# SKIRT/SKIRT9

Hardware: AMD Instinct MI355X
Metric: photon packets/s (whole node), 10^6-cell octree (higher is better)
Workload: dtype f64

## Files before the change

### include/pmc_tuning.h

```cpp
#ifndef PMC_TUNING_H
#define PMC_TUNING_H

#include "pmc.h"

#ifdef __cplusplus
extern "C" {
#endif

int pmc_tuning_set(const char* name, const char* value);
void pmc_tuning_clear(void);

int pmc_set_launch(pmc_ctx* ctx, int32_t block, int32_t grid);

typedef struct pmc_walk_work_values
{
    uint64_t peel_wave_steps, peel_lane_steps, peel_rounds;
    uint64_t prop_wave_steps, prop_lane_steps, prop_rounds;
} pmc_walk_work_values;
int pmc_walk_work(pmc_ctx* ctx, pmc_walk_work_values* out);
typedef struct pmc_debug_table_values
{
    const void* cell_table;
    int64_t cell_slots;
    int64_t loose_base;
    const int32_t* task_cell;
    int64_t num_slots;
} pmc_debug_table_values;
int pmc_debug_tables(pmc_ctx* ctx, pmc_debug_table_values* out);

int pmc_launch_flavour(pmc_ctx* ctx, int32_t* flavour);

int pmc_tune_dipole_cosines(pmc_ctx* ctx, const double* u, int64_t n, double* cos_out);

int pmc_tune_source_velocities(pmc_ctx* ctx, int32_t source, const double* r, int64_t n, double* v_out);


typedef struct pmc_log_geometry_values
{
    int64_t cell_slots, rf_num_lambda, rf_keys, rf_parts, rf_logged;
    int64_t stat_records, stat_parts, stat_logged;
    int64_t chunk, rf_bucket_bits, stat_bucket_bits, scan_threads, sort_block, max_parts, reduce_span, rf_short_run, stat_short_run, max_entries;
} pmc_log_geometry_values;
int pmc_tune_log_geometry(pmc_ctx* ctx, pmc_log_geometry_values* out);

int pmc_tune_log_partition(pmc_ctx* ctx, int32_t stat, int32_t num_parts, const uint32_t* keys, const double* vals, const uint32_t* fills, int64_t n,
                           uint32_t* sorted_keys, double* sorted_vals, uint64_t* start);

int pmc_tune_rf_log_flush(pmc_ctx* ctx, const uint32_t* keys, const double* vals, int64_t n);

int pmc_tune_stat_log_flush(pmc_ctx* ctx, const uint32_t* keys, const double* vals, const uint32_t* fills, int64_t n, double* acc_out);

int pmc_tune_cell_numbering(pmc_ctx* ctx, int32_t* ext_out);


enum
{
    PMC_FN_HG_VALUE = 0,
    PMC_FN_HG_CONE_MEAN = 1,
    PMC_FN_PHASE_VALUE = 2,
    PMC_FN_HG_COSINE = 3,
    PMC_FN_DIPOLE_VALUE = 4,
    PMC_FN_RANDOM_DIRECTION = 5,
    PMC_FN_DIRECTION_ABOUT = 6,
// ... 57 lines not shown
```

### skirt9_amd/csrc/pmc_api.hip

```cpp
#include "pmc_context.h"
#include "pmc_scene_build.h"
#include <memory>

namespace
{
    thread_local std::string t_error;
    constexpr int MAX_DEVICES = 64;
    bool g_slotUsed[MAX_DEVICES][PMC_MAX_CONTEXTS] = {{false}};
    std::mutex g_slotMutex;
}

void pmcSetError(const std::string& message)
{
    t_error = message;
}


extern "C" {

int pmc_abi_version(void)
{
    return PMC_ABI_VERSION;
}

// ... 1 lines not shown
#define PMC_STRINGIFY(x) PMC_STRINGIFY2(x)
#ifndef PMC_BUILD_FLAGS
#define PMC_BUILD_FLAGS "unknown (not built by the Makefile)"
#endif
const char* pmc_build_info(void)
{
    return "libpmc ABI " PMC_STRINGIFY(PMC_ABI_VERSION) ", gfx950, " __VERSION__ ", flags: " PMC_BUILD_FLAGS
#if defined(__FP_FAST_FMA) || defined(__FAST_MATH__)
           " [fast-math macros defined]"
#endif
        ;
}

namespace
{
    __global__ void contractionProbeKernel(double a, double b, double c, double* out) { out[0] = a * b + c; }

    int checkContraction(int device)
    {
        static std::mutex m;
        static bool checked[64] = {false};
        std::lock_guard<std::mutex> lock(m);
        if (device >= 0 && device < 64 && checked[device]) return PMC_OK;
        double* d = nullptr;
        double h = 1.;
        if (hipMalloc(&d, sizeof(double)) != hipSuccess) return fail(PMC_ERR_DEVICE, "hipMalloc failed");
        hipLaunchKernelGGL(contractionProbeKernel, dim3(1), dim3(1), 0, 0, 1. + 0x1p-30, 1. - 0x1p-30, -1., d);
        const hipError_t e = hipMemcpy(&h, d, sizeof(double), hipMemcpyDeviceToHost);
        hipFree(d);
        if (e != hipSuccess) return hipFail(e, "contraction self-test");
        if (h != 0.)
            return fail(PMC_ERR_DEVICE, std::string("this libpmc.so was compiled with floating-point contraction (a * b + c fused): its results would differ from "
                                                    "the reference's in the last bits everywhere; rebuild with -ffp-contract=off.  ") + pmc_build_info());
        if (device >= 0 && device < 64) checked[device] = true;
        return PMC_OK;
    }
}

const char* pmc_last_error(void)
{
    return t_error.c_str();
}

int64_t pmc_frame_layout_of(const pmc_scene* scene, int32_t instrument, pmc_frame_layout* out)
{
    if (!scene) return fail(PMC_ERR_INVALID, "null scene");
    return pmc_layout_compute(scene, instrument, out);
}

void pmc_destroy(pmc_ctx* ctx)
{
    if (!ctx) return;
    hipSetDevice(ctx->device);
    for (int g = 0; g < PMC_MAX_GROUPS; ++g)
    {
        if (ctx->groupStream[g]) hipStreamSynchronize(ctx->groupStream[g]);
        if (ctx->peelStream[g]) hipStreamSynchronize(ctx->peelStream[g]);
    }
    for (void* p : ctx->allocations) hipFree(p);
    for (void* p : ctx->slotAllocations) hipFree(p);
    for (void* p : ctx->segmentAllocations) hipFree(p);
    if (ctx->readback) hipHostFree(ctx->readback);
    for (hipEvent_t e : {ctx->evStart, ctx->evStop})
        if (e) hipEventDestroy(e);
    for (int g = 0; g < PMC_MAX_GROUPS; ++g)
    {
        for (hipEvent_t e : {ctx->evA[g], ctx->evB[g], ctx->evC[g], ctx->evJoin[g], ctx->evProp[g]})
            if (e) hipEventDestroy(e);
        if (g > 0 && ctx->groupStream[g]) hipStreamDestroy(ctx->groupStream[g]);
        if (ctx->peelStream[g]) hipStreamDestroy(ctx->peelStream[g]);
    }
    if (ctx->stream) hipStreamDestroy(ctx->stream);
    if (ctx->slot >= 0)
    {
        std::lock_guard<std::mutex> lock(g_slotMutex);
        g_slotUsed[ctx->device][ctx->slot] = false;
    }
    delete ctx;
}

}

namespace
{
    SceneSwitches readSceneSwitches()
    {
        SceneSwitches sw;
        sw.treeAsBinTree = pmcTune("PMC_TREE_AS_BINTREE") != nullptr;
        sw.noMono = pmcTune("PMC_NO_MONO") != nullptr;
        sw.propNoCheckpoints = pmcTune("PMC_PROP_NO_CHECKPOINTS") != nullptr;
        sw.voroNoPeelKernel = pmcTune("PMC_VORO_NO_PEEL_KERNEL") != nullptr;
        sw.voroNoDeferredScan = pmcTune("PMC_VORO_NO_DEFERRED_SCAN") != nullptr;
        sw.voroNoCull = pmcTune("PMC_VORO_NO_CULL") != nullptr;
        sw.voroNoPropKernel = pmcTune("PMC_VORO_NO_PROP_KERNEL") != nullptr;
        sw.voroNoConeTables = pmcTune("PMC_VORO_NO_CONE_TABLES") != nullptr;
        sw.voroNoObserverLists = pmcTune("PMC_VORO_NO_OBSERVER_LISTS") != nullptr;
        sw.voroConeCullOnly = pmcTune("PMC_VORO_CONE_CULL_ONLY") != nullptr;
        if (const char* v = pmcTune("PMC_VORO_LINK_COUNT_MAX")) sw.voroLinkCountMax = std::min<uint32_t>(sw.voroLinkCountMax, (uint32_t)std::max(0, atoi(v)));
        if (const char* v = pmcTune("PMC_CELL_ORDER")) sw.cellOrderRef = !strcmp(v, "ref");
        if (const char* v = pmcTune("PMC_CELL_SHUFFLE")) sw.cellShuffle = atoi(v);
        if (const char* v = pmcTune("PMC_WALK_BLOCKS_PER_CU")) sw.walkBlocksPerCU = std::max(1, atoi(v));
        if (const char* v = pmcTune("PMC_PEEL_BLOCKS_PER_CU")) sw.peelBlocksPerCU = std::max(1, atoi(v));
        return sw;
    }

    struct DestroyContext
    {
        void operator()(pmc_ctx* ctx) const { pmc_destroy(ctx); }
    };
    using ContextPtr = std::unique_ptr<pmc_ctx, DestroyContext>;

    int makeContext(int device, ContextPtr& made)
    {
        if (device >= MAX_DEVICES) return fail(PMC_ERR_UNSUPPORTED, "device index beyond the context table");
        ContextPtr ctx(new pmc_ctx());
        ctx->device = device;
        {
            std::lock_guard<std::mutex> lock(g_slotMutex);
            for (int sl = 0; sl < PMC_MAX_CONTEXTS && ctx->slot < 0; ++sl)
                if (!g_slotUsed[device][sl])
                {
                    g_slotUsed[device][sl] = true;
                    ctx->slot = sl;
                }
        }
        if (ctx->slot < 0) return fail(PMC_ERR_NOMEM, "too many live pmc contexts (at most " + std::to_string(PMC_MAX_CONTEXTS) + ")");
        auto makeStream = [](hipStream_t* out) { return hipStreamCreateWithPriority(out, hipStreamDefault, 0); };
        if (makeStream(&ctx->stream) != hipSuccess) return fail(PMC_ERR_DEVICE, "hipStreamCreate failed");
        ctx->groupStream[0] = ctx->stream;
        for (int g = 1; g < PMC_MAX_GROUPS; ++g)
            if (makeStream(&ctx->groupStream[g]) != hipSuccess) return fail(PMC_ERR_DEVICE, "hipStreamCreate failed");
        for (int g = 0; g < PMC_MAX_GROUPS; ++g)
            if (makeStream(&ctx->peelStream[g]) != hipSuccess) return fail(PMC_ERR_DEVICE, "hipStreamCreate failed");
        for (hipEvent_t* ev : {&ctx->evStart, &ctx->evStop})
            if (hipEventCreate(ev) != hipSuccess) return fail(PMC_ERR_DEVICE, "hipEventCreate failed");
        for (int g = 0; g < PMC_MAX_GROUPS; ++g)
            for (hipEvent_t* ev : {&ctx->evA[g], &ctx->evB[g], &ctx->evC[g], &ctx->evJoin[g], &ctx->evProp[g]})
                if (hipEventCreate(ev) != hipSuccess) return fail(PMC_ERR_DEVICE, "hipEventCreate failed");
        if (const char* env = getenv("PMC_NUM_GROUPS"))
        {
            ctx->numGroups = std::min(PMC_MAX_GROUPS, std::max(1, atoi(env)));
            ctx->groupsConfigured = true;
        }
        if (hipHostMalloc(reinterpret_cast<void**>(&ctx->readback), PMC_MAX_GROUPS * sizeof(GroupReadback)) != hipSuccess)
            return fail(PMC_ERR_DEVICE, "hipHostMalloc failed");
        made = std::move(ctx);
        return PMC_OK;
    }

    int configureDevice(pmc_ctx* ctx, const SceneSwitches& sw)
    {
        const DevScene& D = ctx->dev;
        if (pmcConfigureKernels(ctx->walkLds, ctx->launchLds) != hipSuccess) return fail(PMC_ERR_DEVICE, "hipFuncSetAttribute failed");
        hipDeviceProp_t prop;
        if (hipGetDeviceProperties(&prop, ctx->device) != hipSuccess) return fail(PMC_ERR_DEVICE, "hipGetDeviceProperties failed");
        ctx->numCU = prop.multiProcessorCount;
        ctx->block = 256;
        ctx->wide = D.grid_kind == PMC_GRID_OCTREE && D.lmax > 10;
        int perCU = pmcWalkBlocksPerCU(D.grid_kind, D.grid_kind == PMC_GRID_OCTREE ? 2 : 0, ctx->wide,
                                       D.grid_kind == PMC_GRID_OCTREE ? pmcPropBlock() : ctx->block, ctx->walkLds);
        if (perCU < 1) perCU = 1;
        if (sw.walkBlocksPerCU) perCU = std::min(perCU, sw.walkBlocksPerCU);
        else perCU = std::min(perCU, D.grid_kind == PMC_GRID_OCTREE ? 1 : 3);
        ctx->grid = ctx->numCU * perCU;
        if (D.grid_kind == PMC_GRID_OCTREE)
        {
            int peelPerCU = pmcWalkBlocksPerCU(D.grid_kind, 1, ctx->wide, pmcPeelBlock(), ctx->walkLds);
            peelPerCU = std::min(std::max(peelPerCU, 1), 1);
            if (sw.peelBlocksPerCU) peelPerCU = sw.peelBlocksPerCU;
            ctx->peelGrid = ctx->numCU * peelPerCU;
        }
        ctx->numSlots = 24 * 1024 * 1024;
        if (const char* env = getenv("PMC_NUM_SLOTS"))
        {
            ctx->numSlots = std::max<int64_t>(1024, atoll(env));
            ctx->slotsConfigured = true;
        }
        return PMC_OK;
    }
}

extern "C" {

int pmc_create(const pmc_scene* scene, int32_t device, pmc_ctx** out)
{
    return pmc_create_ext(scene, nullptr, device, out);
}

int pmc_create_ext(const pmc_scene* scene, const pmc_scene_ext* ext, int32_t device, pmc_ctx** out)
{
    if (!scene || !out) return fail(PMC_ERR_INVALID, "null argument");
    *out = nullptr;
    int rc = PMC_OK;
    SceneExtension extension;
    if ((rc = checkScene(*scene, ext, extension))) return rc;
    if (pmcExperimentBuild())
    {
        static std::atomic<bool> said{false};
        if (!said.exchange(true)) fprintf(stderr, "libpmc: this library was built with an ablation / perturbation macro (a tuning experiment): its results are NOT those of the engine\n");
    }
    int count = 0;
    if (hipGetDeviceCount(&count) != hipSuccess || count < 1)
        return fail(PMC_ERR_DEVICE, "no HIP device available: the MI355X engine cannot run (there is no CPU fallback)");
    if (device < 0 || device >= count) return fail(PMC_ERR_INVALID, "invalid device index");
    HIP_TRY(hipSetDevice(device));
    if ((rc = checkContraction(device))) return rc;

    ContextPtr ctx;
    if ((rc = makeContext(device, ctx))) return rc;
    const SceneSwitches switches = readSceneSwitches();
    SceneTables tables;
    if ((rc = buildSceneTables(*scene, extension, switches, *ctx, ctx->dev, tables))) return rc;
    ctx->frameSize = tables.frameSize;
    ctx->rfSize = tables.rfSize;
    ctx->frames = ctx->dev.frames;
    ctx->walkLds = tables.lds.walkBytes, ctx->transitionLds = tables.lds.transitionBytes, ctx->launchLds = tables.lds.launchBytes;
    if ((rc = configureDevice(ctx.get(), switches))) return rc;
    *out = ctx.release();
    return PMC_OK;
}

int pmc_set_launch(pmc_ctx* ctx, int32_t block, int32_t grid)
{
    if (!ctx) return fail(PMC_ERR_INVALID, "null context");
    if (block > 0)
    {
        if (block % 64 || block > 256) return fail(PMC_ERR_INVALID, "block must be a multiple of 64 and at most 256");
        ctx->block = block;
    }
    if (grid > 0) ctx->grid = grid;
    return PMC_OK;
}

int pmc_set_num_slots(pmc_ctx* ctx, int64_t num_slots)
{
    if (!ctx) return fail(PMC_ERR_INVALID, "null context");
    if (num_slots < 1 || num_slots > (int64_t(1) << 30)) return fail(PMC_ERR_INVALID, "num_slots out of range");
    ctx->numSlots = num_slots;
    ctx->slotsConfigured = true;
    return PMC_OK;
}

int pmc_bind_frames(pmc_ctx* ctx, double* device_ptr, int64_t num_doubles)
{
    if (!ctx || !device_ptr) return fail(PMC_ERR_INVALID, "null argument");
    if (num_doubles != ctx->frameSize) return fail(PMC_ERR_INVALID, "frame buffer size mismatch");
    ctx->frames = device_ptr;
    ctx->dev.frames = device_ptr;
    ctx->sceneDirty = true;
    return PMC_OK;
}

int pmc_clear_frames(pmc_ctx* ctx)
{
    if (!ctx) return fail(PMC_ERR_INVALID, "null context");
    HIP_TRY(hipSetDevice(ctx->device));
    HIP_TRY(hipMemsetAsync(ctx->frames, 0, size_t(ctx->frameSize) * sizeof(double), ctx->stream));
    return PMC_OK;
}

int pmc_set_progress(pmc_ctx* ctx, pmc_progress_fn report, void* user, double interval_seconds)
{
    if (!ctx) return fail(PMC_ERR_INVALID, "null context");
    ctx->progress = report;
    ctx->progressUser = user;
    ctx->progressInterval = interval_seconds > 0. ? interval_seconds : 0.;
    return PMC_OK;
}

int pmc_sync(pmc_ctx* ctx)
{
    if (!ctx) return fail(PMC_ERR_INVALID, "null context");
    HIP_TRY(hipSetDevice(ctx->device));
    HIP_TRY(hipStreamSynchronize(ctx->stream));
    return PMC_OK;
}

int pmc_last_kernel_ms(pmc_ctx* ctx, float* ms)
{
    if (!ctx || !ms) return fail(PMC_ERR_INVALID, "null argument");
    if (!ctx->timed) return fail(PMC_ERR_INVALID, "no segment has been run yet");
    *ms = ctx->walkMs;
    return PMC_OK;
// ... 165 lines not shown
```

### skirt9_amd/csrc/pmc_context.h

```cpp
#ifndef PMC_CONTEXT_H
#define PMC_CONTEXT_H

#include "pmc_tables.h"
#include "../../include/pmc_layout.h"
#include "../../include/pmc_tuning.h"
#include <hip/hip_runtime.h>
#include <algorithm>
#include <chrono>
#include <cmath>
#include <cstdio>
#include <rccl/rccl.h>
#include <cstdlib>
#include <cstring>
#include <deque>
#include <atomic>
#include <mutex>
#include <string>
#include <thread>
#include <map>
#include <vector>

extern "C" const char* pmcTune(const char* name);
extern "C" hipError_t pmcUploadScene(int slot, const DevScene* scene, hipStream_t stream);
extern "C" hipError_t pmcConfigureKernels(size_t walkLds, size_t transitionLds);
// ... 28 lines not shown
extern "C" hipError_t pmcLaunchSourceVelocities(int slot, int source, const double* r, int64_t n, double* out, hipStream_t stream);
extern "C" hipError_t pmcLaunchDeviceFunction(int slot, int function, const double* args, int widthIn, int64_t n, double* out, int widthOut, hipStream_t stream);
extern "C" hipError_t pmcLaunchLocate(int kind, const double* nodes, int numNodes, const double* x, int64_t n, int32_t* out, hipStream_t stream);
extern "C" hipError_t pmcLaunchDetector(int slot, int instrument, const double* r, int64_t n, int32_t* pixel, int32_t* inside, hipStream_t stream);
extern "C" hipError_t pmcLaunchWavelengthBins(int slot, int instrument, const double* lambda, int64_t n, int32_t* ell, hipStream_t stream);
extern "C" hipError_t pmcLaunchAngularProbabilities(int slot, int source, const double* k, int64_t n, double* out, hipStream_t stream);
extern "C" hipError_t pmcLaunchTransition(int slot, int flavour, int slotBase, int numSlots, int group, uint64_t seed, const int* list, int listLen, int maxBlocks,
                                          size_t ldsBytes, const StatLogArgs* statLog, uint64_t count, hipStream_t stream);
extern "C" hipError_t pmcLaunchLaunch(int slot, int flavour, int slotBase, int numSlots, int group, uint64_t first, uint64_t count, uint64_t seed, int initial,
                                      int maxBlocks, size_t ldsBytes, const StatLogArgs* statLog, hipStream_t stream);
extern "C" hipError_t pmcLaunchStatFlush(int slot, const uint32_t* keys, const double* vals, uint32_t* sortedKeys, double* sortedVals, unsigned long long n,
                                         int numParts, void* temp, int numCU, const uint32_t* chunkFill, hipStream_t stream);
extern "C" int pmcStatBucketBits();
extern "C" void pmcLogConstants(pmc_log_geometry_values* out);
extern "C" hipError_t pmcLaunchLogPartition(int stat, const uint32_t* keys, const double* vals, uint32_t* sortedKeys, double* sortedVals, unsigned long long n,
                                            int numParts, void* temp, int numCU, const uint32_t* fills, hipStream_t stream);
extern "C" hipError_t pmcLaunchCycleStart(int slot, int gridKind, int kin, int slotBase, int numSlots, int listCounter, int* listOut, const int* listIn,
                                          int listLen, int maxBlocks, size_t ldsBytes, const PeelSortArgs* sort, hipStream_t stream);
extern "C" hipError_t pmcLaunchTrace(int slot, int gridKind, int wide, int uniform, const double r[3], const double k[3],
                                     const double* kdev, int32_t* m, double* ds, int32_t cap, int32_t* n, size_t ldsBytes,
                                     hipStream_t stream);
extern "C" int pmcProbeWorkWords(void);
extern "C" hipError_t pmcLaunchIntegrate(int slot, int gridKind, int wide, int averaged, const double* origins, const double* directions, const double* q,
                                         double* sums, unsigned long long numRays, unsigned long long* work, int grid, size_t ldsBytes, hipStream_t stream);
extern "C" hipError_t pmcLaunchLocateCells(int slot, int gridKind, int wide, const double* positions, int32_t* walkCells, int32_t* cells,
                                           unsigned long long numPoints, int grid, size_t ldsBytes, hipStream_t stream);
extern "C" hipError_t pmcLaunchGatherCells(const int32_t* walkCells, const double* q, double* values, unsigned long long numPoints, int numValues, int grid,
                                           hipStream_t stream);

namespace
{
    inline int hipFail(hipError_t e, const char* what)
    {
        return fail(PMC_ERR_DEVICE, std::string(what) + ": " + hipGetErrorString(e));
    }
}

#define HIP_TRY(call)                                           \
    do                                                          \
    {                                                           \
        hipError_t e_ = (call);                                 \
        if (e_ != hipSuccess) return hipFail(e_, #call);        \
    } while (0)

struct GroupReadback
{
    unsigned long long live;
    unsigned long long rfLogFill;
    unsigned long long statLogFill;
    unsigned long long historyCursor;
    unsigned long long statFreeBlocks;
};

struct pmc_ctx final : TableSink
{
    int device{0};
    int slot{-1};
    bool sceneDirty{true};
    hipStream_t stream{nullptr};
    int numGroups{3};
    hipStream_t groupStream[PMC_MAX_GROUPS]{};
    hipStream_t peelStream[PMC_MAX_GROUPS]{};
    hipEvent_t evA[PMC_MAX_GROUPS]{}, evB[PMC_MAX_GROUPS]{}, evC[PMC_MAX_GROUPS]{}, evJoin[PMC_MAX_GROUPS]{}, evProp[PMC_MAX_GROUPS]{};
    hipEvent_t evStart{nullptr}, evStop{nullptr};
    bool timed{false};
    float totalMs{0}, walkMs{0}, transitionMs{0};
    float peelMs{0}, propMs{0};
    int generations{0};
    float integrateMs{0};
    unsigned long long integrateLaneSteps{0}, integrateWaveSteps{0};
    float temperatureMs{0};
    float sampleMs{0};
    DevScene dev{};
    std::vector<void*> allocations;
    std::vector<void*> slotAllocations;
    double* frames{nullptr};
    int64_t frameSize{0};
    int64_t rfSize{0};
    size_t walkLds{0}, transitionLds{0}, launchLds{0};
    int block{256};
    int grid{0};
    int peelGrid{0};
    int wide{0};
    int numCU{256};
    int64_t numSlots{0};
    int64_t allocatedSlots{0};
    GroupReadback* readback{nullptr};
    unsigned long long internalErrorsSeen{0};
    pmc_progress_fn progress{nullptr};
    void* progressUser{nullptr};
    double progressInterval{3.};
    size_t steppedDownFree{0};
    bool slotsConfigured{false};
    bool groupsConfigured{false};
    unsigned long long overflowsSeen{0};
    int32_t* statPoolIota{nullptr};
    int64_t statPoolBlocks{0};
    int statPoolGrowths{0};
    std::vector<void*> segmentAllocations;
    uint32_t* rfKeys[PMC_MAX_GROUPS][2]{};
    double* rfVals[PMC_MAX_GROUPS][2]{};
    unsigned long long rfCap[PMC_MAX_GROUPS]{};
    void* rfTemp[PMC_MAX_GROUPS]{};
    PeelRec* peelRec[PMC_MAX_GROUPS][PMC_SORT_OBS]{};
    int32_t* peelList[PMC_MAX_GROUPS][PMC_SORT_OBS]{};
    void* peelTemp[PMC_MAX_GROUPS][PMC_SORT_OBS]{};
    unsigned long long* xcdCursors{nullptr};
    int peelCap[PMC_MAX_GROUPS]{};
    size_t rfTempBytes{0};
    uint32_t* statKeys[PMC_MAX_GROUPS][2]{};
    double* statVals[PMC_MAX_GROUPS][2]{};
    unsigned long long statCap[PMC_MAX_GROUPS]{};
    void* statTemp[PMC_MAX_GROUPS]{};
// ... 170 lines not shown
```

### skirt9_amd/csrc/pmc_run.hip

```cpp
#include "pmc_context.h"

namespace
{
    int allocateSlotArrays(pmc_ctx* ctx, int64_t n);
    void releaseSlots(pmc_ctx* ctx)
    {
        for (void* p : ctx->slotAllocations) hipFree(p);
        ctx->slotAllocations.clear();
        ctx->allocatedSlots = 0;
    }

    int allocateSlots(pmc_ctx* ctx, int64_t n)
    {
        hipSetDevice(ctx->device);
        releaseSlots(ctx);
        ctx->planning = true;
        ctx->plannedBytes = 0;
        int rc = allocateSlotArrays(ctx, n);
        ctx->planning = false;
        if (rc) return rc;
        size_t freeBytes = 0, totalBytes = 0;
        if (!ctx->slotsConfigured && n > (int64_t(1) << 20) && hipMemGetInfo(&freeBytes, &totalBytes) == hipSuccess && ctx->plannedBytes > freeBytes / 2)
        {
            const int64_t less = std::max<int64_t>(int64_t(1) << 20, n / 2);
// ... 154 lines not shown
        bool poolGrows;
        int statInstruments;
        int launchFlavour;
        int launchBlocks, cycleBlocks, transitionBlocks;
        int voroPropGrid, voroPeelGrid, voroPropSegments;
        bool serialWalks, genDump, xcdAffinity, voroPeelKernels, voroPropKernel, voroWalksInSeries;
    };
    struct SegmentRun
    {
        bool active[PMC_MAX_GROUPS], haveWalk[PMC_MAX_GROUPS];
        bool listBuilt[PMC_MAX_GROUPS];
        int listHalf[PMC_MAX_GROUPS];
        bool peelSorted[PMC_MAX_GROUPS];
        bool poolCannotGrow;
        float walkMs, transMs, peelMs, propMs;
        int generations;
    };

    int provisionSlots(pmc_ctx* ctx, uint64_t count, int* numSlots)
    {
        const int64_t want = std::min<int64_t>(ctx->numSlots, (int64_t)std::min<uint64_t>(count, uint64_t(1) << 30));
        bool grow = want > ctx->allocatedSlots;
        if (grow && ctx->allocatedSlots > 0 && ctx->steppedDownFree)
        {
            size_t freeBytes = 0, totalBytes = 0;
            grow = hipMemGetInfo(&freeBytes, &totalBytes) == hipSuccess && freeBytes > ctx->steppedDownFree + ctx->steppedDownFree / 4;
        }
        if (grow)
        {
            HIP_TRY(hipStreamSynchronize(ctx->stream));
            ctx->steppedDownFree = 0;
            int rc = allocateSlots(ctx, want);
            if (rc) return rc;
        }
        *numSlots = (int)std::min<int64_t>(want, ctx->allocatedSlots);
        HIP_TRY(sceneUpToDate(ctx));
        return PMC_OK;
    }

    int launchFlavour(const pmc_ctx* ctx)
    {
        const DevScene& D = ctx->dev;
        if (pmcTune("PMC_LAUNCH_GENERIC") != nullptr) return D.kin ? PMC_LAUNCH_KIN : 0;
        return pmcLaunchFlavourOf(D.src, D.num_sources, D.kin);
    }

    SegmentPlan planSegment(const pmc_ctx* ctx, int numSlots, uint64_t first, uint64_t count, uint64_t seed)
    {
        const DevScene& D = ctx->dev;
        SegmentPlan P;
        std::memset(&P, 0, sizeof(P));
        P.first = first, P.count = count, P.seed = seed;
        P.octree = D.grid_kind == PMC_GRID_OCTREE;
        P.serialWalks = pmcTune("PMC_SERIAL_WALKS") != nullptr;
        P.genDump = pmcTune("PMC_GEN_DUMP") != nullptr;
        const bool peelSort = pmcTune("PMC_NO_PEEL_SORT") == nullptr;
        int G = ctx->numGroups;
        if (numSlots < G * 65536) G = 1;
        {
            int observers = 0;
            for (int i = 0; i < D.num_instruments; ++i) observers += D.inst[i].same_observer ? 0 : 1;
            if (D.grid_kind == PMC_GRID_VORONOI && observers <= PMC_SORT_OBS && !ctx->groupsConfigured && peelSort) G = 1;
        }
        P.G = G;
        const int per = ((numSlots + G - 1) / G + PMC_TRANSITION_ALIGN - 1) / PMC_TRANSITION_ALIGN * PMC_TRANSITION_ALIGN;
        for (int g = 0; g < G; ++g)
        {
            P.base[g] = std::min(numSlots, g * per);
            P.size[g] = std::min(per, numSlots - P.base[g]);
        }
        P.walkFlavour = (D.rf_store ? 1 : 0) | (D.explicit_absorption ? 2 : 0) | (D.num_media > 1 ? 4 : 0);
        P.peelForm = (ctx->wide ? 1 : 0) | (D.num_media > 1 ? 2 : 0);
        if (pmcPeelHasQueues(P.peelForm, ctx->walkLds)) P.peelForm |= 4;
        P.propCheckpoints = pmcPropHasCheckpoints(P.walkFlavour, ctx->walkLds);
        P.propSortIndex = -1;
        if (peelSort && (!P.octree || (P.peelForm & 4)))
        {
            int observers = 0;
            for (int i = 0; i < D.num_instruments; ++i)
                if (!D.inst[i].same_observer)
                {
                    if (observers < PMC_SORT_OBS) P.sortObs[observers] = i;
                    ++observers;
                }
            if (observers <= PMC_SORT_OBS) P.numSortObs = observers;
        }
        if (!P.octree && P.numSortObs > 0 && P.numSortObs < PMC_SORT_OBS && pmcTune("PMC_NO_PROP_SORT") == nullptr) P.propSortIndex = P.numSortObs;
        P.numSortLists = P.numSortObs + (P.propSortIndex >= 0 ? 1 : 0);
        PeelSortArgs& sa = P.sortArgs;
        sa.numObs = P.numSortObs;
        sa.propIndex = P.propSortIndex;
        for (int i = 0; i < 16; ++i) sa.sortIndex[i] = -1;
        for (int k = 0; k < P.numSortObs; ++k) sa.obs[k] = P.sortObs[k], sa.sortIndex[P.sortObs[k]] = (int8_t)k;
        const double gdx = D.gx1 - D.gx0, gdy = D.gy1 - D.gy0, gdz = D.gz1 - D.gz0;
        sa.centre[0] = 0.5 * (D.gx0 + D.gx1), sa.centre[1] = 0.5 * (D.gy0 + D.gy1), sa.centre[2] = 0.5 * (D.gz0 + D.gz1);
        sa.scale = PMC_PEEL_TILES / std::sqrt(gdx * gdx + gdy * gdy + gdz * gdz);
        P.xcdAffinity = pmcTune("PMC_NO_XCD_AFFINITY") == nullptr;
        P.sparseLists = P.octree && pmcTune("PMC_NO_LIVE_LISTS") == nullptr;
        P.listTasksPerLane = 1;
        if (const char* env = pmcTune("PMC_LIST_TASKS_PER_LANE")) P.listTasksPerLane = std::max(1, atoi(env));
        P.voroPeelKernels = D.grid_kind == PMC_GRID_VORONOI && pmcTune("PMC_VORO_NO_PEEL_KERNEL") == nullptr;
        P.voroPropKernel = D.grid_kind == PMC_GRID_VORONOI && D.vgen_run && pmcTune("PMC_VORO_NO_PROP_KERNEL") == nullptr
                           && !(pmcTune("PMC_VORO_PLAIN_PROP_ONLY") && (D.num_media > 1 || D.rf_store || D.explicit_absorption));
        P.voroWalksInSeries = pmcTune("PMC_VORO_WALKS_IN_SERIES") != nullptr;
        P.voroPropSegments = (P.xcdAffinity && pmcTune("PMC_VPROP_XCD_SEGMENTS")) ? 8 : 1;
        int propBlocks = pmcVoroPropWavesPerSimd(), peelBlocks = pmcVoroPeelWavesPerSimd();
        if (const char* v = pmcTune("PMC_VPROP_BLOCKS_PER_CU")) propBlocks = std::max(1, atoi(v));
        if (const char* v = pmcTune("PMC_VPEEL_BLOCKS_PER_CU")) peelBlocks = std::max(1, atoi(v));
        P.voroPropGrid = ctx->numCU * propBlocks, P.voroPeelGrid = ctx->numCU * peelBlocks;
        const LogPlan logs = pmcLogPlan(ctx);
        P.rfLogged = logs.rfLogged;
        if (D.rf_store && P.octree && logs.rfParts > pmcRfMaxParts())
        {
            static std::atomic<bool> said{false};
            if (!said.exchange(true))
                fprintf(stderr, "libpmc: the radiation field table has %lld entries, more than the log's counting sort partitions (%d x %d): contributions are added atomically\n",
// ... 799 lines not shown
```

### skirt9_amd/engine.py

```python
import ctypes as C
import os

import numpy as np

from .host import AdaptiveMesh, CounterValues, DustHeating, FrameLayout, SceneExt, SceneHead, heating_struct, mesh_struct

_LIBDIR = os.path.join(os.path.dirname(os.path.abspath(__file__)), "lib")

SYMBOLS = ["pmc_abi_version", "pmc_build_info", "pmc_last_error", "pmc_frame_layout_of", "pmc_create", "pmc_create_ext", "pmc_destroy", "pmc_bind_frames",
           "pmc_clear_frames", "pmc_run_primary", "pmc_set_progress", "pmc_sync", "pmc_download", "pmc_frames_device", "pmc_frames_size",
           "pmc_last_kernel_ms", "pmc_counters", "pmc_reset_counters", "pmc_trace_ray", "pmc_integrate_rays",
           "pmc_last_integrate_work", "pmc_integrate_weighted_rays", "pmc_sample_cells", "pmc_last_sample_ms", "pmc_dust_temperatures",
           "pmc_last_temperature_ms", "pmc_set_launch",
           "pmc_set_num_slots", "pmc_last_timing", "pmc_last_walk_timing", "pmc_walk_work", "pmc_radiation_field_size", "pmc_radiation_field_device",
           "pmc_download_radiation_field", "pmc_clear_radiation_field", "pmc_bind_radiation_field", "pmc_sampler_create",
           "pmc_sampler_density", "pmc_sampler_destroy", "pmc_sampler_create_mesh", "pmc_history_range", "pmc_comm_init_all", "pmc_comm_unique_id",
           "pmc_comm_init_rank", "pmc_comm_size", "pmc_comm_destroy", "pmc_reduce_frames", "pmc_allreduce_radiation_field",
           "pmc_debug_tables", "pmc_tuning_set", "pmc_tuning_clear", "pmc_tune_dipole_cosines", "pmc_tune_source_velocities",
           "pmc_launch_flavour", "pmc_tune_log_geometry", "pmc_tune_log_partition", "pmc_tune_rf_log_flush", "pmc_tune_stat_log_flush",
           "pmc_tune_cell_numbering", "pmc_tune_device_function", "pmc_tune_device_function_widths", "pmc_tune_locate", "pmc_tune_instrument",
           "pmc_tune_detector", "pmc_tune_wavelength_bins", "pmc_tune_angular_probabilities", "pmc_tune_walk_cycle", "pmc_tune_walk_cycle_limits"]

DEVICE_FUNCTIONS = {"hg_value": 0, "hg_cone_mean": 1, "phase_value": 2, "hg_cosine": 3, "dipole_value": 4, "random_direction": 5, "direction_about": 6,
                    "lambert_lower_branch": 7, "generalized_exp": 8, "interpolate_loglog": 9, "lnmean": 10, "peel_taumax": 11, "shifted_wavelength": 12}
LOCATE_KINDS = {"locate": 0, "locate_clip": 1, "locate_basic": 2}

_lib = None


class DebugTables(C.Structure):
    _fields_ = [("cell_table", C.c_void_p), ("cell_slots", C.c_int64), ("loose_base", C.c_int64), ("task_cell", C.c_void_p), ("num_slots", C.c_int64)]


class WalkWork(C.Structure):
    _fields_ = [(n, C.c_uint64) for n in ("peel_wave_steps", "peel_lane_steps", "peel_rounds", "prop_wave_steps",
                                          "prop_lane_steps", "prop_rounds")]


class InstrumentValues(C.Structure):
    _fields_ = ([(n, C.c_double) for n in ("costheta", "sintheta", "cosphi", "sinphi", "cosomega", "sinomega", "xpmin", "xpsiz", "ypmin", "ypsiz",
                                           "aperture_r2", "zp1")]
                + [(n, C.c_int64) for n in ("nxp", "nyp", "num_border", "num_lambda", "include_sed", "include_ifu")])


class LogGeometry(C.Structure):
    _fields_ = [(n, C.c_int64) for n in ("cell_slots", "rf_num_lambda", "rf_keys", "rf_parts", "rf_logged", "stat_records", "stat_parts", "stat_logged",
                                         "chunk", "rf_bucket_bits", "stat_bucket_bits", "scan_threads", "sort_block", "max_parts", "reduce_span",
                                         "rf_short_run", "stat_short_run", "max_entries")]


class WalkCycleIn(C.Structure):
    _fields_ = ([("n", C.c_int64), ("live_list", C.c_int32)]
                + [(n, C.c_void_p) for n in ("list", "r", "k", "mask", "ppW", "u1", "u2", "depth", "hint", "nscatt", "wavelength", "dust_ext", "dust_sca",
                                             "dust_abs", "dust_idx", "W", "rfell")])


class WalkCycleOut(C.Structure):
    _fields_ = ([(n, C.c_void_p) for n in ("ptau", "sint", "nint", "mint", "taupath", "tausample")]
                + [(n, C.c_uint64) for n in ("visits", "rewalks", "paths", "internal_errors")])


def lib():
    global _lib
    if _lib is None:
        path = os.environ.get("PMC_LIBRARY") or os.path.join(_LIBDIR, "libpmc.so")
        if not os.path.exists(path):
            raise RuntimeError(f"{path} is missing: the HIP engine has not been built (run `make` or "
                               "__graft_entry__.build()); there is no CPU fallback")
        L = C.CDLL(path)
        L.pmc_abi_version.restype = C.c_int
        L.pmc_last_error.restype = C.c_char_p
        L.pmc_build_info.restype = C.c_char_p
        L.pmc_frame_layout_of.restype = C.c_int64
        L.pmc_frame_layout_of.argtypes = [C.c_void_p, C.c_int32, C.POINTER(FrameLayout)]
        L.pmc_create.argtypes = [C.c_void_p, C.c_int32, C.POINTER(C.c_void_p)]
        if hasattr(L, "pmc_create_ext"):
            L.pmc_create_ext.argtypes = [C.c_void_p, C.c_void_p, C.c_int32, C.POINTER(C.c_void_p)]
            L.pmc_tune_dipole_cosines.argtypes = [C.c_void_p, C.c_void_p, C.c_int64, C.c_void_p]
        if hasattr(L, "pmc_tune_source_velocities"):
            L.pmc_tune_source_velocities.argtypes = [C.c_void_p, C.c_int32, C.c_void_p, C.c_int64, C.c_void_p]
        L.pmc_destroy.argtypes = [C.c_void_p]
        L.pmc_bind_frames.argtypes = [C.c_void_p, C.c_void_p, C.c_int64]
        L.pmc_clear_frames.argtypes = [C.c_void_p]
        L.pmc_run_primary.argtypes = [C.c_void_p, C.c_uint64, C.c_uint64, C.c_uint64]
        L.pmc_sync.argtypes = [C.c_void_p]
        L.pmc_download.argtypes = [C.c_void_p, C.c_void_p, C.c_int64]
        L.pmc_frames_device.restype = C.c_void_p
        L.pmc_frames_device.argtypes = [C.c_void_p]
        L.pmc_frames_size.restype = C.c_int64
# ... 62 lines not shown
            L.pmc_tune_angular_probabilities.argtypes = [C.c_void_p, C.c_int32, C.c_void_p, C.c_int64, C.c_void_p, C.POINTER(C.c_int32), C.c_void_p,
                                                         C.POINTER(C.c_double)]
        if hasattr(L, "pmc_tune_walk_cycle"):
            L.pmc_tune_walk_cycle.argtypes = [C.c_void_p, C.POINTER(WalkCycleIn), C.POINTER(WalkCycleOut)]
            L.pmc_tune_walk_cycle_limits.argtypes = [C.c_void_p, C.POINTER(C.c_int64), C.POINTER(C.c_int32), C.POINTER(C.c_int32), C.POINTER(C.c_int32)]
        _lib = L
    return _lib


INTEGRATE_PASS_VALUES = 4
INTEGRATE_BATCH_RAYS = 1 << 22
SAMPLE_CHUNK_POINTS = 1 << 20

ENVIRONMENT_SETTINGS = ("PMC_NUM_SLOTS", "PMC_NUM_GROUPS", "PMC_STAT_POOL_BLOCKS")


def set_tuning(name, value="1"):
    L = lib()
    if hasattr(L, "pmc_tuning_set"):
        _check(L.pmc_tuning_set(name.encode(), None if value is None else str(value).encode()))
    elif value is None:
        os.environ.pop(name, None)
    else:
        os.environ[name] = str(value)


def clear_tuning():
    L = lib()
    if hasattr(L, "pmc_tuning_clear"):
        L.pmc_tuning_clear()


def tuning_from_environment():
    for key, value in os.environ.items():
        if key.startswith("PMC_") and key not in ENVIRONMENT_SETTINGS and key != "PMC_LIBRARY":
            set_tuning(key, value)


def _ptr(array):
    return None if array is None else array.ctypes.data_as(C.c_void_p)


def _check(rc):
    if rc != 0:
        raise RuntimeError(f"pmc error {rc}: {lib().pmc_last_error().decode()}")


def history_range(num_packets, rank, num_ranks):
    first, count = C.c_uint64(0), C.c_uint64(0)
    lib().pmc_history_range(int(num_packets), int(rank), int(num_ranks), C.byref(first), C.byref(count))
    return int(first.value), int(count.value)


class Communicator:

    def __init__(self, handles):
        self.handles = handles

    @classmethod
    def all(cls, devices):
        n = len(devices)
        dev = (C.c_int32 * n)(*devices)
        out = (C.c_void_p * n)()
        _check(lib().pmc_comm_init_all(n, dev, out))
        return cls([C.c_void_p(h) for h in out])

    @staticmethod
    def unique_id():
        buf = C.create_string_buffer(128)
        _check(lib().pmc_comm_unique_id(buf))
        return buf.raw

    @classmethod
    def rank(cls, device, num_ranks, rank, unique_id):
        out = C.c_void_p()
        _check(lib().pmc_comm_init_rank(device, num_ranks, rank, C.c_char_p(unique_id), C.byref(out)))
        return cls([out])

    def size(self, index=0):
        n, me = C.c_int32(0), C.c_int32(0)
        _check(lib().pmc_comm_size(self.handles[index], C.byref(n), C.byref(me)))
        return int(n.value), int(me.value)

    def close(self):
        for h in self.handles:
            lib().pmc_comm_destroy(h)
        self.handles = []


class Particles(C.Structure):
    _fields_ = [("kernel", C.c_int32), ("num_particles", C.c_int64), ("particle", C.POINTER(C.c_double)), ("num_blocks", C.c_int32),
                ("xgrid", C.POINTER(C.c_double)), ("ygrid", C.POINTER(C.c_double)), ("zgrid", C.POINTER(C.c_double)),
                ("block_start", C.POINTER(C.c_int64)), ("block_list", C.POINTER(C.c_int32))]


KERNEL_CUBIC_SPLINE, KERNEL_UNIFORM = 1, 2


class _Sampler:
    _h = None

    def density(self, positions):
        r = np.ascontiguousarray(positions, dtype=np.float64).reshape(-1, 3)
        out = np.empty(r.shape[0], dtype=np.float64)
        _check(lib().pmc_sampler_density(self._h, _ptr(r), r.shape[0], _ptr(out)))
        return out
# ... 417 lines not shown
```

Measured before the change: 211.3 million.

## Plan stream creation around hardware queue count and default to two groups

Replaces the fixed set of eight streams (four group streams plus four peel streams) with a stream plan derived from the number of hardware queues (GPU_MAX_HW_QUEUES, default 4) and the group count. With enough queues, group and side-walk streams are created in an order that spreads each group and its side stream across different hardware queues. With too few queues, the plan falls back to serial walks without side streams. The default group count also drops from three to two. The aim is to stop streams aliasing onto the same hardware queue and serialising, at the cost of less concurrency from fewer groups.

```diff
diff --git a/include/pmc_tuning.h b/include/pmc_tuning.h
--- a/include/pmc_tuning.h
+++ b/include/pmc_tuning.h
@@ -9,6 +9,27 @@
 
 int pmc_tuning_set(const char* name, const char* value);
 void pmc_tuning_clear(void);
+
+#define PMC_STREAM_PLAN_MAX_GROUPS 4
+#define PMC_HARDWARE_QUEUES_VARIABLE "GPU_MAX_HW_QUEUES"
+enum
+{
+    PMC_STREAM_PLAN_DEFAULT = 0,
+    PMC_STREAM_PLAN_EIGHT = 1,
+    PMC_STREAM_PLAN_SHARED_SIDE = 2,
+    PMC_STREAM_PLAN_SERIAL = 3,
+    PMC_STREAM_PLAN_INTERLEAVED = 4,
+    PMC_STREAM_PLAN_TWO_GROUPS = 5
+};
+typedef struct pmc_stream_plan_values
+{
+    int32_t plan;
+    int32_t num_groups, num_group_streams, num_side_streams;
+    int32_t side_of_group[PMC_STREAM_PLAN_MAX_GROUPS];
+    int32_t num_streams;
+    int32_t order[2 * PMC_STREAM_PLAN_MAX_GROUPS], queue[2 * PMC_STREAM_PLAN_MAX_GROUPS], queue_measured[2 * PMC_STREAM_PLAN_MAX_GROUPS];
+} pmc_stream_plan_values;
+int pmc_stream_plan(int32_t plan, int32_t groups, int32_t side_walks, int32_t queues, pmc_stream_plan_values* out);
 
 int pmc_set_launch(pmc_ctx* ctx, int32_t block, int32_t grid);
 
diff --git a/skirt9_amd/csrc/pmc_api.hip b/skirt9_amd/csrc/pmc_api.hip
--- a/skirt9_amd/csrc/pmc_api.hip
+++ b/skirt9_amd/csrc/pmc_api.hip
@@ -77,11 +77,7 @@
 {
     if (!ctx) return;
     hipSetDevice(ctx->device);
-    for (int g = 0; g < PMC_MAX_GROUPS; ++g)
-    {
-        if (ctx->groupStream[g]) hipStreamSynchronize(ctx->groupStream[g]);
-        if (ctx->peelStream[g]) hipStreamSynchronize(ctx->peelStream[g]);
-    }
+    for (hipStream_t s : ctx->streams) hipStreamSynchronize(s);
     for (void* p : ctx->allocations) hipFree(p);
     for (void* p : ctx->slotAllocations) hipFree(p);
     for (void* p : ctx->segmentAllocations) hipFree(p);
@@ -92,10 +88,8 @@
     {
         for (hipEvent_t e : {ctx->evA[g], ctx->evB[g], ctx->evC[g], ctx->evJoin[g], ctx->evProp[g]})
             if (e) hipEventDestroy(e);
-        if (g > 0 && ctx->groupStream[g]) hipStreamDestroy(ctx->groupStream[g]);
-        if (ctx->peelStream[g]) hipStreamDestroy(ctx->peelStream[g]);
-    }
-    if (ctx->stream) hipStreamDestroy(ctx->stream);
+    }
+    for (hipStream_t s : ctx->streams) hipStreamDestroy(s);
     if (ctx->slot >= 0)
     {
         std::lock_guard<std::mutex> lock(g_slotMutex);
@@ -150,18 +144,8 @@
                 }
         }
         if (ctx->slot < 0) return fail(PMC_ERR_NOMEM, "too many live pmc contexts (at most " + std::to_string(PMC_MAX_CONTEXTS) + ")");
-        auto makeStream = [](hipStream_t* out) { return hipStreamCreateWithPriority(out, hipStreamDefault, 0); };
-        if (makeStream(&ctx->stream) != hipSuccess) return fail(PMC_ERR_DEVICE, "hipStreamCreate failed");
-        ctx->groupStream[0] = ctx->stream;
-        for (int g = 1; g < PMC_MAX_GROUPS; ++g)
-            if (makeStream(&ctx->groupStream[g]) != hipSuccess) return fail(PMC_ERR_DEVICE, "hipStreamCreate failed");
-        for (int g = 0; g < PMC_MAX_GROUPS; ++g)
-            if (makeStream(&ctx->peelStream[g]) != hipSuccess) return fail(PMC_ERR_DEVICE, "hipStreamCreate failed");
         for (hipEvent_t* ev : {&ctx->evStart, &ctx->evStop})
             if (hipEventCreate(ev) != hipSuccess) return fail(PMC_ERR_DEVICE, "hipEventCreate failed");
-        for (int g = 0; g < PMC_MAX_GROUPS; ++g)
-            for (hipEvent_t* ev : {&ctx->evA[g], &ctx->evB[g], &ctx->evC[g], &ctx->evJoin[g], &ctx->evProp[g]})
-                if (hipEventCreate(ev) != hipSuccess) return fail(PMC_ERR_DEVICE, "hipEventCreate failed");
         if (const char* env = getenv("PMC_NUM_GROUPS"))
         {
             ctx->numGroups = std::min(PMC_MAX_GROUPS, std::max(1, atoi(env)));
@@ -170,6 +154,45 @@
         if (hipHostMalloc(reinterpret_cast<void**>(&ctx->readback), PMC_MAX_GROUPS * sizeof(GroupReadback)) != hipSuccess)
             return fail(PMC_ERR_DEVICE, "hipHostMalloc failed");
         made = std::move(ctx);
+        return PMC_OK;
+    }
+
+    int makeStreams(pmc_ctx* ctx)
+    {
+        const DevScene& D = ctx->dev;
+        int groups = ctx->numGroups;
+        if (D.grid_kind == PMC_GRID_VORONOI && !ctx->groupsConfigured)
+        {
+            int observers = 0;
+            for (int i = 0; i < D.num_instruments; ++i) observers += D.inst[i].same_observer ? 0 : 1;
+            if (observers <= PMC_SORT_OBS) groups = 1;
+        }
+        const bool sideWalks = D.grid_kind == PMC_GRID_OCTREE || D.grid_kind == PMC_GRID_VORONOI;
+        const char* named = pmcTune("PMC_STREAM_PLAN");
+        pmcStreamPlan(named ? atoi(named) : PMC_STREAM_PLAN_DEFAULT, groups, sideWalks, pmcHardwareQueues(), ctx->plan);
+        const pmc_stream_plan_values& plan = ctx->plan;
+        hipStream_t side[PMC_MAX_GROUPS] = {};
+        ctx->streams.reserve(size_t(plan.num_streams));
+        for (int i = 0; i < plan.num_streams; ++i)
+        {
+            hipStream_t s = nullptr;
+            if (hipStreamCreateWithPriority(&s, hipStreamDefault, 0) != hipSuccess) return fail(PMC_ERR_DEVICE, "hipStreamCreate failed");
+            ctx->streams.push_back(s);
+            const int which = plan.order[i];
+            if (which < PMC_MAX_GROUPS)
+            {
+                if (which < plan.num_group_streams) ctx->groupStream[which] = s;
+            }
+            else
+                side[which - PMC_MAX_GROUPS] = s;
+        }
+        ctx->stream = ctx->groupStream[0];
+        for (int g = 0; g < plan.num_groups; ++g)
+        {
+            if (plan.side_of_group[g] >= 0) ctx->peelStream[g] = side[plan.side_of_group[g]];
+            for (hipEvent_t* ev : {&ctx->evA[g], &ctx->evB[g], &ctx->evC[g], &ctx->evJoin[g], &ctx->evProp[g]})
+                if (hipEventCreate(ev) != hipSuccess) return fail(PMC_ERR_DEVICE, "hipEventCreate failed");
+        }
         return PMC_OK;
     }
 
@@ -240,6 +263,7 @@
     ctx->rfSize = tables.rfSize;
     ctx->frames = ctx->dev.frames;
     ctx->walkLds = tables.lds.walkBytes, ctx->transitionLds = tables.lds.transitionBytes, ctx->launchLds = tables.lds.launchBytes;
+    if ((rc = makeStreams(ctx.get()))) return rc;
     if ((rc = configureDevice(ctx.get(), switches))) return rc;
     *out = ctx.release();
     return PMC_OK;
@@ -254,6 +278,13 @@
         ctx->block = block;
     }
     if (grid > 0) ctx->grid = grid;
+    return PMC_OK;
+}
+
+int pmc_stream_plan(int32_t plan, int32_t groups, int32_t side_walks, int32_t queues, pmc_stream_plan_values* out)
+{
+    if (!out) return fail(PMC_ERR_INVALID, "null argument");
+    pmcStreamPlan(plan, groups, side_walks != 0, queues, *out);
     return PMC_OK;
 }
 
diff --git a/skirt9_amd/csrc/pmc_context.h b/skirt9_amd/csrc/pmc_context.h
--- a/skirt9_amd/csrc/pmc_context.h
+++ b/skirt9_amd/csrc/pmc_context.h
@@ -104,13 +104,112 @@
     unsigned long long statFreeBlocks;
 };
 
+static_assert(PMC_STREAM_PLAN_MAX_GROUPS == PMC_MAX_GROUPS, "include/pmc_tuning.h and pmc_device.h disagree on the number of slot groups");
+constexpr int PMC_STREAM_PLAN_FEW_QUEUES = PMC_STREAM_PLAN_SERIAL;
+
+inline void pmcMeasuredQueues(int n, int queues, int32_t* queue)
+{
+    int load[64] = {0};
+    const int Q = std::min(64, std::max(1, queues));
+    load[0] = 1;
+    for (int i = 0; i < n; ++i)
+    {
+        int q = -1;
+        for (int k = 0; k < Q && q < 0; ++k)
+            if (load[k] == 0) q = k;
+        if (q < 0)
+        {
+            q = 0;
+            for (int k = 1; k < Q; ++k)
+                if (load[k] <= load[q]) q = k;
+        }
+        ++load[q];
+        queue[i] = q;
+    }
+}
+
+inline void pmcStreamPlan(int plan, int groups, bool sideWalks, int queues, pmc_stream_plan_values& out)
+{
+    const int Q = std::max(1, queues);
+    int G = std::min(PMC_STREAM_PLAN_MAX_GROUPS, std::max(1, groups));
+    if (plan < PMC_STREAM_PLAN_DEFAULT || plan > PMC_STREAM_PLAN_TWO_GROUPS) plan = PMC_STREAM_PLAN_DEFAULT;
+    if (plan == PMC_STREAM_PLAN_DEFAULT) plan = Q >= 2 * G ? PMC_STREAM_PLAN_INTERLEAVED : PMC_STREAM_PLAN_FEW_QUEUES;
+    if (plan == PMC_STREAM_PLAN_TWO_GROUPS) G = std::min(G, 2);
+    out = pmc_stream_plan_values{};
+    out.plan = plan;
+    out.num_groups = G;
+    out.num_group_streams = G;
+    for (int g = 0; g < PMC_STREAM_PLAN_MAX_GROUPS; ++g) out.side_of_group[g] = -1;
+    const int SIDE = PMC_STREAM_PLAN_MAX_GROUPS;
+    int n = 0;
+    auto groupStreams = [&](int count) { for (int g = 0; g < count; ++g) out.order[n++] = g; };
+    if (plan == PMC_STREAM_PLAN_EIGHT)
+    {
+        groupStreams(PMC_STREAM_PLAN_MAX_GROUPS);
+        for (int s = 0; s < PMC_STREAM_PLAN_MAX_GROUPS; ++s) out.order[n++] = SIDE + s;
+        if (sideWalks)
+        {
+            out.num_side_streams = G;
+            for (int g = 0; g < G; ++g) out.side_of_group[g] = g;
+        }
+    }
+    else if (sideWalks && plan == PMC_STREAM_PLAN_SHARED_SIDE)
+    {
+        groupStreams(G);
+        out.num_side_streams = 1;
+        out.order[n++] = SIDE;
+        for (int g = 0; g < G; ++g) out.side_of_group[g] = 0;
+    }
+    else if (sideWalks && (plan == PMC_STREAM_PLAN_INTERLEAVED || plan == PMC_STREAM_PLAN_TWO_GROUPS))
+    {
+        out.num_side_streams = G;
+        for (int g = 0; g < G; ++g) out.side_of_group[g] = g;
+        int32_t perm[2 * PMC_STREAM_PLAN_MAX_GROUPS], rr[2 * PMC_STREAM_PLAN_MAX_GROUPS], ms[2 * PMC_STREAM_PLAN_MAX_GROUPS];
+        n = 2 * G;
+        for (int g = 0; g < G; ++g) perm[g] = g, perm[G + g] = SIDE + g;
+        for (int i = 0; i < n; ++i) rr[i] = i % Q;
+        pmcMeasuredQueues(n, Q, ms);
+        long best = -1;
+        do
+        {
+            int at[2 * PMC_STREAM_PLAN_MAX_GROUPS] = {0};
+            for (int i = 0; i < n; ++i) at[perm[i]] = i;
+            long score = 0;
+            for (int g = 0; g < G; ++g)
+            {
+                score += 1000 * (rr[at[g]] == rr[at[SIDE + g]]) + 100 * (ms[at[g]] == ms[at[SIDE + g]]);
+                for (int h = g + 1; h < G; ++h) score += 10 * (ms[at[g]] == ms[at[h]]) + (rr[at[g]] == rr[at[h]]);
+            }
+            if (best < 0 || score < best)
+            {
+                best = score;
+                for (int i = 0; i < n; ++i) out.order[i] = perm[i];
+            }
+        } while (std::next_permutation(perm + 1, perm + n));
+    }
+    else
+        groupStreams(G);
+    out.num_streams = n;
+    for (int i = 0; i < n; ++i) out.queue[i] = i % Q;
+    pmcMeasuredQueues(n, Q, out.queue_measured);
+}
+
+inline int pmcHardwareQueues()
+{
+    const char* env = getenv(PMC_HARDWARE_QUEUES_VARIABLE);
+    const int q = env ? atoi(env) : 0;
+    return q > 0 ? q : 4;
+}
+
 struct pmc_ctx final : TableSink
 {
     int device{0};
     int slot{-1};
     bool sceneDirty{true};
     hipStream_t stream{nullptr};
-    int numGroups{3};
+    int numGroups{2};
+    pmc_stream_plan_values plan{};
+    std::vector<hipStream_t> streams;
     hipStream_t groupStream[PMC_MAX_GROUPS]{};
     hipStream_t peelStream[PMC_MAX_GROUPS]{};
     hipEvent_t evA[PMC_MAX_GROUPS]{}, evB[PMC_MAX_GROUPS]{}, evC[PMC_MAX_GROUPS]{}, evJoin[PMC_MAX_GROUPS]{}, evProp[PMC_MAX_GROUPS]{};
diff --git a/skirt9_amd/csrc/pmc_run.hip b/skirt9_amd/csrc/pmc_run.hip
--- a/skirt9_amd/csrc/pmc_run.hip
+++ b/skirt9_amd/csrc/pmc_run.hip
@@ -230,7 +230,7 @@
         std::memset(&P, 0, sizeof(P));
         P.first = first, P.count = count, P.seed = seed;
         P.octree = D.grid_kind == PMC_GRID_OCTREE;
-        P.serialWalks = pmcTune("PMC_SERIAL_WALKS") != nullptr;
+        P.serialWalks = pmcTune("PMC_SERIAL_WALKS") != nullptr || ctx->plan.num_side_streams == 0;
         P.genDump = pmcTune("PMC_GEN_DUMP") != nullptr;
         const bool peelSort = pmcTune("PMC_NO_PEEL_SORT") == nullptr;
         int G = ctx->numGroups;
@@ -240,6 +240,7 @@
             for (int i = 0; i < D.num_instruments; ++i) observers += D.inst[i].same_observer ? 0 : 1;
             if (D.grid_kind == PMC_GRID_VORONOI && observers <= PMC_SORT_OBS && !ctx->groupsConfigured && peelSort) G = 1;
         }
+        G = std::min(G, int(ctx->plan.num_groups));
         P.G = G;
         const int per = ((numSlots + G - 1) / G + PMC_TRANSITION_ALIGN - 1) / PMC_TRANSITION_ALIGN * PMC_TRANSITION_ALIGN;
         for (int g = 0; g < G; ++g)
diff --git a/skirt9_amd/engine.py b/skirt9_amd/engine.py
--- a/skirt9_amd/engine.py
+++ b/skirt9_amd/engine.py
@@ -11,7 +11,7 @@
            "pmc_clear_frames", "pmc_run_primary", "pmc_set_progress", "pmc_sync", "pmc_download", "pmc_frames_device", "pmc_frames_size",
            "pmc_last_kernel_ms", "pmc_counters", "pmc_reset_counters", "pmc_trace_ray", "pmc_integrate_rays",
            "pmc_last_integrate_work", "pmc_integrate_weighted_rays", "pmc_sample_cells", "pmc_last_sample_ms", "pmc_dust_temperatures",
-           "pmc_last_temperature_ms", "pmc_set_launch",
+           "pmc_last_temperature_ms", "pmc_set_launch", "pmc_stream_plan",
            "pmc_set_num_slots", "pmc_last_timing", "pmc_last_walk_timing", "pmc_walk_work", "pmc_radiation_field_size", "pmc_radiation_field_device",
            "pmc_download_radiation_field", "pmc_clear_radiation_field", "pmc_bind_radiation_field", "pmc_sampler_create",
            "pmc_sampler_density", "pmc_sampler_destroy", "pmc_sampler_create_mesh", "pmc_history_range", "pmc_comm_init_all", "pmc_comm_unique_id",
@@ -35,6 +35,11 @@
 class WalkWork(C.Structure):
     _fields_ = [(n, C.c_uint64) for n in ("peel_wave_steps", "peel_lane_steps", "peel_rounds", "prop_wave_steps",
                                           "prop_lane_steps", "prop_rounds")]
+
+
+class StreamPlan(C.Structure):
+    _fields_ = [("plan", C.c_int32), ("num_groups", C.c_int32), ("num_group_streams", C.c_int32), ("num_side_streams", C.c_int32),
+                ("side_of_group", C.c_int32 * 4), ("num_streams", C.c_int32), ("order", C.c_int32 * 8), ("queue", C.c_int32 * 8), ("queue_measured", C.c_int32 * 8)]
 
 
 class InstrumentValues(C.Structure):
@@ -203,6 +208,16 @@
     return int(first.value), int(count.value)
 
 
+def stream_plan(plan, groups, side_walks, queues):
+    out = StreamPlan()
+    L = lib()
+    L.pmc_stream_plan.argtypes = [C.c_int32, C.c_int32, C.c_int32, C.c_int32, C.POINTER(StreamPlan)]
+    _check(L.pmc_stream_plan(int(plan), int(groups), 1 if side_walks else 0, int(queues), C.byref(out)))
+    return {"plan": out.plan, "num_groups": out.num_groups, "num_group_streams": out.num_group_streams, "num_side_streams": out.num_side_streams,
+            "side_of_group": list(out.side_of_group)[:out.num_groups], "num_streams": out.num_streams,
+            "order": list(out.order)[:out.num_streams], "queue": list(out.queue)[:out.num_streams], "queue_measured": list(out.queue_measured)[:out.num_streams]}
+
+
 class Communicator:
 
     def __init__(self, handles):
```

Result: no change. 213.2 million, median of 6 (+0.9%).
